# cvxopt/smcp

Measured on AMD Instinct MI355X. Metric: Newton KKT solves/sec, higher is better.
Workload: dtype f64; 1 GPU; synth50k nested block-arrow SDP n=50000, 8073 cliques, m=100; kktsolver=chol, n=50000, cliques=8073, m=100, blkval_doubles=2493568, update_doubles=10689536, parallelism=single

## Files before the change

### smcp_amd/build.py

```python
import os
import shutil
import subprocess
import sys

HERE = os.path.dirname(os.path.abspath(__file__))
CSRC = os.path.join(HERE, "csrc")
LIB = os.path.join(HERE, "libsmcp_amd.so")
SOURCES = ["capi.hip", "symbolic.cpp"]
DEPS = ["front_large.hip", "front_mfma.hip", "capi.hip", "kkt.hip", "kkt_qr.hip", "front_generic.hip", "front_mrc.hip", "front_edm.hip", "wgblas.hpp", "context.hpp", "symbolic.cpp",
        "symbolic.hpp", "../../include/smcp_amd.h"]


def _stale():
    if not os.path.exists(LIB):
        return True
    t = os.path.getmtime(LIB)
    for d in os.listdir(CSRC):
        if os.path.getmtime(os.path.join(CSRC, d)) > t:
            return True
    return os.path.getmtime(os.path.join(HERE, "..", "include", "smcp_amd.h")) > t


def build(force=False, verbose=True):
    if not force and not _stale():
        return LIB
    hipcc = shutil.which("hipcc") or "/opt/rocm/bin/hipcc"
    cmd = [hipcc, "--offload-arch=gfx950", "-O3", "-std=c++17", "-fPIC", "-shared",
           "-Wno-unused-result", "-Wno-unused-value", "-pthread", "-o", LIB] + [os.path.join(CSRC, s) for s in SOURCES]
    if os.environ.get("SMCP_STAMPS") == "1":
        cmd.insert(1, "-DSMCP_STAMPS")
    for flag in os.environ.get("SMCP_CXXFLAGS", "").split():
        cmd.insert(1, flag)
    if verbose:
        print(" ".join(cmd), file=sys.stderr)
    subprocess.check_call(cmd)
    return LIB


if __name__ == "__main__":
    build(force="--force" in sys.argv)
```

### smcp_amd/csrc/capi.hip

```cpp
#include <hip/hip_runtime.h>
#include <memory>
#include <unordered_map>

#include <algorithm>
#include <chrono>
#include <cstdio>
#include <cstring>
#include <map>
#include <new>
#include <atomic>
#include <thread>
#include <type_traits>
#include <vector>

#include "../../include/smcp_amd.h"
#include "context.hpp"
#include "switches.hpp"
#include "front_generic.hip"
#include "front_mfma.hip"
#include "front_large.hip"
#include "front_inv.hip"
#include "front_n16.hip"
#include "front_downfam.hip"
#include "front_fam.hip"
#include "front_fam2.hip"
#include "front_lfsp.hip"
#include "front_leafgram.hip"
#include "front_famt.hip"
#include "front_flow.hip"
#include "front_mrc.hip"
#include "front_edm.hip"

using namespace smcp;

#define HIPCHK(x)                                                                        \
  do {                                                                                   \
    hipError_t e_ = (x);                                                                 \
    if (e_ != hipSuccess) {                                                              \
      fprintf(stderr, "smcp_amd: HIP error %s at %s:%d\n", hipGetErrorString(e_), __FILE__, __LINE__); \
      return SMCP_EHIP;                                                                  \
    }                                                                                    \
  } while (0)

namespace {

enum {
  KID_chol_level = 0, KID_llt_level, KID_pinv_level, KID_gather_level, KID_completion_all,
  KID_hess_up_level, KID_hess_down_level, KID_hess_down_inv_all, KID_hess_up_inv_level, KID_scale_an,
  KID_factor_yaa, KID_trsm_fwd_level, KID_trsm_bwd_level, KID_amap, KID_aadj, KID_scatter_constraints,
  KID_dense_potrf, KID_dense_potrs, KID_vec_axpby, KID_axpby, KID_reduce_cliques, KID_reduce_final,
  KID_hess_up_mfma, KID_hess_down_mfma, KID_chol_mfma, KID_pinv_mfma, KID_prep_lk,
  KID_hess_up_mfma_hbm, KID_hess_down_mfma_hbm, KID_chol_mfma_hbm, KID_pinv_mfma_hbm,
  KID_gram_partial, KID_gram_reduce, KID_hess_up_pad,
  KID_lf_assemble, KID_lf_clear_upd, KID_lf_up1, KID_lf_up2, KID_lf_up3, KID_lf_down1, KID_lf_down2, KID_lf_down3,
  KID_lf_pinv1, KID_lf_pinv2, KID_lf_diag, KID_lf_chol_panel, KID_lf_chol_trail, KID_lf_pack_upd,
  KID_lf_prep_s, KID_lf_prep_row, KID_lf_prep_k, KID_factor_yaa_lds,
  KID_factor_inverse, KID_hess_down_inv_mfma, KID_hess_down_inv_mfma_hbm, KID_hess_up_inv_mfma, KID_hess_up_inv_mfma_hbm,
  KID_completion_mfma, KID_completion_mfma_hbm, KID_lf_copy_an, KID_lf_ri_an, KID_lf_dinv1, KID_lf_dinv2,
  KID_lf_uinv1, KID_lf_uinv2, KID_lf_completion, KID_hess_up_n16, KID_llt_mfma, KID_llt_mfma_hbm, KID_lf_llt,
  KID_hess_up_fam, KID_qr_rmul, KID_qr_dots, KID_qr_comb, KID_qr_small, KID_fam2_prep, KID_mid_chol, KID_lf_diag_inv, KID_lfsp_up, KID_lfsp_prep, KID_leaf_gram, KID_leaf_tables, KID_fam_sparse, KID_gram_diag128, KID_lf_assemble_lds, KID_fam_terms, KID_famt_prep, KID_lf_assemble_lds_dyn, KID_lf_zsp, KID_fam_terms_grp, KID_lf_assemble_fz, KID_factor_inverse_lds, KID_chol_flow,
  KID_mrc_diag, KID_mrc_rank, KID_mrc_reduce, KID_mrc_factor, KID_cut_signs, KID_cut_weights,
  KID_edm_rank, KID_edm_reduce, KID_edm_factor, KID_edm_dense, KID_hess_down_fam,
  KID_COUNT
};
const char* const KID_NAMES[KID_COUNT] = {
  "k_chol_level", "k_llt_level", "k_pinv_level", "k_gather_level", "k_completion_all",
  "k_hess_up_level", "k_hess_down_level", "k_hess_down_inv_all", "k_hess_up_inv_level", "k_scale_an",
  "k_factor_yaa", "k_trsm_fwd_level", "k_trsm_bwd_level", "k_amap", "k_aadj", "k_scatter_constraints",
  "k_dense_potrf", "k_dense_potrs", "k_vec_axpby", "k_axpby", "k_reduce_cliques", "k_reduce_final",
  "k_hess_up_mfma<true>", "k_hess_down_mfma<true>", "k_chol_mfma<true>", "k_pinv_mfma<true>", "k_prep_lk",
  "k_hess_up_mfma<false>", "k_hess_down_mfma<false>", "k_chol_mfma<false>", "k_pinv_mfma<false>",
  "k_gram_partial", "k_gram_reduce", "k_hess_up_pad",
  "k_lf_assemble", "k_lf_clear_upd", "k_lf_up1", "k_lf_up2", "k_lf_up3", "k_lf_down1", "k_lf_down2", "k_lf_down3",
  "k_lf_pinv1", "k_lf_pinv2", "k_lf_diag", "k_lf_chol_panel", "k_lf_chol_trail", "k_lf_pack_upd",
  "k_lf_prep_s", "k_lf_prep_row", "k_lf_prep_k", "k_factor_yaa_lds",
  "k_factor_inverse", "k_hess_down_inv_mfma<true>", "k_hess_down_inv_mfma<false>", "k_hess_up_inv_mfma<true>",
  "k_hess_up_inv_mfma<false>", "k_completion_mfma<true>", "k_completion_mfma<false>", "k_lf_copy_an", "k_lf_ri_an",
  "k_lf_dinv1", "k_lf_dinv2", "k_lf_uinv1", "k_lf_uinv2", "k_lf_completion", "k_hess_up_n16",
  "k_llt_mfma<true>", "k_llt_mfma<false>", "k_lf_llt", "k_hess_up_fam",
  "k_stack_trsm", "k_stack_dots", "k_stack_comb", "k_qr_small", "k_fam2_prep", "k_mid_chol", "k_lf_diag_inv", "k_lfsp_up", "k_lfsp_prep", "k_leaf_pairs", "k_leaf_tables", "k_fam_sparse", "k_gram_diag128", "k_lf_assemble_lds", "k_fam_terms", "k_famt_prep", "k_lf_assemble_lds_dyn", "k_lf_zsp", "k_fam_terms_grp", "k_lf_assemble_fz", "k_factor_inverse_lds", "k_chol_flow",
  "k_mrc_diag", "k_mrc_rank", "k_mrc_reduce", "k_mrc_factor", "k_cut_signs", "k_cut_weights",
  "k_edm_rank", "k_edm_reduce", "k_edm_factor", "k_edm_dense", "k_hess_down_fam"};

inline void note_launch(csp_ctx* c, int kid) {
  const hipError_t e = hipGetLastError();
  if (e != hipSuccess && !c->launch_err) {
    c->launch_err = (int)e;
    fprintf(stderr, "smcp_amd: launch of %s failed: %s\n", (kid >= 0 && kid < KID_COUNT) ? KID_NAMES[kid] : "?", hipGetErrorString(e));
  }
}
inline hipError_t end_call(csp_ctx* c) {
  hipError_t e = hipGetLastError();
  if (e == hipSuccess && c->launch_err) e = c->launch_err > 0 ? (hipError_t)c->launch_err : hipErrorLaunchFailure;
  c->launch_err = 0;
  return e;
}

__global__ void k_race_spin(long long ticks) {
  const long long t0 = wall_clock64();
  for (int it = 0; it < (1 << 22) && wall_clock64() - t0 < ticks; ++it) __builtin_amdgcn_s_sleep(8);
}
struct RaceInject {
  std::atomic<uint64_t> state{0};
  std::atomic<int64_t> injected{0};
  std::atomic<int> max_us{200};
  std::atomic<int> drop_joins{0};
  bool on() const { return state.load(std::memory_order_relaxed) != 0; }
  void seed(uint64_t s) { state.store(s ? (s * 0x9E3779B97F4A7C15ull) | 1ull : 0ull); }
  uint64_t next() {
    uint64_t x = state.load(std::memory_order_relaxed);
    x ^= x << 13; x ^= x >> 7; x ^= x << 17;
    state.store(x | 1ull, std::memory_order_relaxed);
    return x;
  }
};
inline RaceInject& race_inject() {
  static RaceInject r;
  static const bool init = [] { const char* e = sw_str("SMCP_RACE"); if (e && atoll(e) > 0) r.seed((uint64_t)atoll(e)); return true; }();
  (void)init;
  return r;
}
inline void race_delay(hipStream_t s, bool always = true) {
  RaceInject& r = race_inject();
  if (!r.on()) return;
  const uint64_t x = r.next();
  if (!always && (x >> 40) % 4 != 0) return;
  const long long us = 5 + (long long)((x >> 16) % (uint64_t)std::max(1, r.max_us.load(std::memory_order_relaxed) - 4));
  hipLaunchKernelGGL(k_race_spin, dim3(1), dim3(64), 0, s, us * 100);
  r.injected.fetch_add(1, std::memory_order_relaxed);
}

inline unsigned sync_event_flags() {
  static int sys = -1;
  if (sys < 0) { const char* e = sw_str("SMCP_EVENT_SYSFENCE"); sys = (e && e[0] == '1') ? 1 : 0; }
  return sys ? hipEventDisableTiming : (hipEventDisableTiming | hipEventReleaseToDevice);
// ... 1061 lines not shown
  if (!D.sp_rt) {
    if (dev_alloc(&D.sp_rt, std::max<int64_t>(c->S.updlen(), 1), D.bytes)) return false;
    if (dev_alloc(&D.sp_mk, std::max<int64_t>(c->S.blklen(), 1), D.bytes)) return false;
  }
  MfmaArgs b = a;
  b.sp_rt = D.sp_rt; b.sp_mk = D.sp_mk;
  if (D.sp_fac_gen != D.fac_gen || D.sp_lk_gen != D.lk_gen) {
    MfmaArgs p = b;
    p.t.lev = D.lfsp_list;
    launch(c, KID_lfsp_prep, k_lfsp_prep, dim3((unsigned)D.lfsp_cnt), dim3(256), st, p, a.ysc, D.sp_rt, D.sp_mk);
    D.sp_fac_gen = D.fac_gen; D.sp_lk_gen = D.lk_gen;
  }
  static int gdiv = -1;
  if (gdiv < 0) { const char* e = sw_str("SMCP_LFSP_G"); gdiv = e ? std::max(1, atoi(e)) : 1; }
  const int g = std::max(1, (nrhs + gdiv - 1) / gdiv);
  const dim3 grid(g, cnt), blk(256);
  const bool grouped = grp && grp->ngroups > 0;
  MfmaArgs bg = b;
  if (grouped) { bg.grp_ptr = grp->ptr; bg.grp_list = grp->list; }
  const dim3 ggrid(g, grouped ? grp->ngroups : cnt);
  static const int gocc = sw_int("SMCP_LFSP_OCC", 2);
  if (grouped && gocc == 1) {
    if (exact) {
      launch(c, KID_lfsp_up, k_lfsp_up<8, 4, 1, 3, 1, false, true>, grid, blk, st, b, U, ldu);
      launch(c, KID_lfsp_up, k_lfsp_up<8, 4, 2, 1, 1, false, true, true>, ggrid, blk, st, bg, U, ldu);
      launch(c, KID_lfsp_up, k_lfsp_up<8, 4, 4, 4, 1, false, true>, grid, blk, st, b, U, ldu);
    } else {
      launch(c, KID_lfsp_up, k_lfsp_up<8, 4, 1, 3, 1, false, false>, grid, blk, st, b, U, ldu);
      launch(c, KID_lfsp_up, k_lfsp_up<8, 4, 2, 1, 1, false, false, true>, ggrid, blk, st, bg, U, ldu);
      launch(c, KID_lfsp_up, k_lfsp_up<8, 4, 4, 4, 1, false, false>, grid, blk, st, b, U, ldu);
    }
    return true;
  }
  if (exact) {
    launch(c, KID_lfsp_up, k_lfsp_up<8, 4, 1, 3, 1, false, true>, grid, blk, st, b, U, ldu);
    if (grouped) launch(c, KID_lfsp_up, k_lfsp_up<8, 4, 2, 2, 1, false, true, true>, ggrid, blk, st, bg, U, ldu);
    else launch(c, KID_lfsp_up, k_lfsp_up<8, 4, 2, 2, 1, false, true>, grid, blk, st, b, U, ldu);
    launch(c, KID_lfsp_up, k_lfsp_up<8, 4, 4, 4, 1, false, true>, grid, blk, st, b, U, ldu);
  } else {
    launch(c, KID_lfsp_up, k_lfsp_up<8, 4, 1, 3, 1, false, false>, grid, blk, st, b, U, ldu);
    if (grouped) launch(c, KID_lfsp_up, k_lfsp_up<8, 4, 2, 2, 1, false, false, true>, ggrid, blk, st, bg, U, ldu);
    else launch(c, KID_lfsp_up, k_lfsp_up<8, 4, 2, 2, 1, false, false>, grid, blk, st, b, U, ldu);
    launch(c, KID_lfsp_up, k_lfsp_up<8, 4, 4, 4, 1, false, false>, grid, blk, st, b, U, ldu);
  }
  return true;
}
bool lfsp_dynamic_ok(csp_ctx* c, const MfmaArgs& a) {
  static int on = -1;
  if (on < 0) { const char* e = sw_str("SMCP_LFSP"); on = (e && e[0] == '0') ? 0 : 1; }
  const DeviceCtx& D = c->D;
  return on && a.kc_ptr && a.ymode == 2 && a.ysc && D.kc_maxlist_large > 0 && D.kc_maxlist_large <= LFSP_ECAP && D.lfsp_cnt;
}

void hess_up_fast(csp_ctx* c, double* U, int nrhs, int64_t ldu, const double* ysc, int ymode, hipStream_t st, int set = 0,
                  int64_t sparse_j0 = -1, const int32_t* ids = nullptr, int64_t lev_lo = 0, int64_t lev_hi = -1,
                  const double* yroot = nullptr) {
  MfmaArgs a0 = mfma_args(c, ysc, ymode, nrhs);
  const bool sparse = sparse_j0 >= 0 && c->D.kc_ptr;
  if (sparse) {
    a0.kc_ptr = c->D.kc_ptr; a0.kc_off = c->D.kc_off; a0.kc_val = c->D.kc_val; a0.kc_ids = ids;
    a0.kc_stride = (int)(c->D.m + 1); a0.kc_j0 = (int)sparse_j0;
  }
  const bool groups_on = sparse && set == 0 && c->lfsp_any_groups && c->D.lfsp_skip && lfsp_dynamic_ok(c, a0);
  const bool fgroups_on = sparse && set == 0 && c->famt_any_groups && c->D.famt_skip && !famt_disabled() && !fam2_disabled() && c->D.lg_request &&
                          c->D.kc_ij && a0.ymode == 2 && a0.ysc && c->D.fam_maxterms <= FAMT_TCAP / 2 &&
                          c->D.cnnz <= (int64_t)4 * c->S.nsn * std::max<int64_t>(1, c->D.m);
  if (groups_on || fgroups_on) a0.chskip = groups_on && fgroups_on ? c->D.both_skip : (groups_on ? c->D.lfsp_skip : c->D.famt_skip);
  c->fz_live = false;
  {
    static int fzenv = -1;
    if (fzenv < 0) { const char* e = sw_str("SMCP_FZ"); fzenv = (e && e[0] == '0') ? 0 : 1; }
    bool want = fzenv && sparse && (set == 0 || (set == 1 && c->fz_set1_ok)) && lev_lo == 0 && lev_hi < 0 && !fgroups_on && c->D.fz_ok && !famt_disabled() && !fam2_disabled() &&
                c->D.lg_request && c->D.kc_ij && a0.ymode == 2 && a0.ysc && famt_terms_ok(c->D) &&
                c->D.cnnz <= (int64_t)4 * c->S.nsn * std::max<int64_t>(1, c->D.m) && !use_generic(c) && use_large() && c->D.gp_tptr;
    int famlevels = 0, nofill = 0;
    if (want) {
      for (int64_t l = 0; l < c->S.nlev; ++l)
        for_level_classes(c, l, a0, [&](bool lds, MfmaArgs a, int cnt, size_t, int) {
          if (lds && a.nS > 0 && a.level > 0) ++famlevels;
          if (!lds && (size_t)a.level < c->fz_levels.size() && c->fz_levels[(size_t)a.level] && !(a.nchmax > 0 && lf_assemble_fills(c, a, cnt, nrhs, true))) { want = false; ++nofill; }
        }, set);
      if (famlevels != 1) want = false;
    }
    if (want) { a0.fz_on = 1; a0.fz_no = c->D.fz_no; }
    static int occ = -1;
    if (occ < 0) occ = sw_on("SMCP_OCC", 0);
    if (occ && sparse)
      fprintf(stderr, "fz: want %d famlevels %d nofill %d nlev %d (env %d set %d lev %d..%d fgroups %d fz_ok %d famt_off %d fam2_off %d lg_request %d kc_ij %d ymode %d ysc %d maxterms %d cnnz %lld nsn %lld m %lld generic %d nrhs %d)\n",
              (int)want, famlevels, nofill, (int)c->S.nlev, fzenv, set, (int)lev_lo, (int)lev_hi, (int)fgroups_on, (int)c->D.fz_ok, (int)famt_disabled(), (int)fam2_disabled(), (int)c->D.lg_request,
              c->D.kc_ij != nullptr, a0.ymode, a0.ysc != nullptr, (int)c->D.fam_maxterms, (long long)c->D.cnnz, (long long)c->S.nsn, (long long)c->D.m, (int)use_generic(c), nrhs);
  }
  auto dense_input_on = [&](MfmaArgs& a, int cnt, double* Ub, int nr, hipStream_t s) {
    if (!sparse) return;
    for (int r0 = 0; r0 < nr; r0 += 65535) {
      MfmaArgs af = a;
      af.kc_j0 = a.kc_j0 + r0;
      const int64_t pan = (int64_t)(a.nnmax + a.namax) * a.nnmax;
      const int nz = (int)std::max<int64_t>(1, std::min<int64_t>(std::min<int64_t>(a.nnmax, 64), pan / 16384));
      launch(c, KID_scatter_constraints, k_panel_fill, dim3(cnt, std::min(65535, nr - r0), nz), dim3(256), s, af, Ub + (int64_t)r0 * ldu, ldu);
    }
    a.kc_ptr = nullptr;
  };
  auto dense_input = [&](MfmaArgs& a, int cnt) { dense_input_on(a, cnt, U, nrhs, st); };
  for (int64_t l = lev_lo; l < (lev_hi < 0 ? c->S.nlev : lev_hi); ++l) {
    for_level_classes(c, l, a0, [&](bool lds, MfmaArgs a, int cnt, size_t bytes, int thr) {
      static int fam_minrhs = -1;
      if (fam_minrhs < 0) { const char* e = sw_str("SMCP_FAM_MINRHS"); fam_minrhs = e ? atoi(e) : 1; }
      if (lds && a.nS > 0 && (sparse || nrhs >= fam_minrhs)) {
        const int nS = a.nS;
        a.nS = 0;
        if (a.level > 0) {
          MfmaArgs af = a;
          af.t.lev = a.t.lev + (cnt - nS);
          if (fgroups_on && (size_t)l < c->famt_grp.size() && c->famt_grp[(size_t)l].ngroups > 0) {
            af.grp_ptr = c->famt_grp[(size_t)l].ptr; af.grp_list = c->famt_grp[(size_t)l].list; af.famt_ngrp = c->famt_grp[(size_t)l].ngroups;
          }
          if (!try_fam(c, af, nS, nrhs, U, ldu, st)) {
            fprintf(stderr, "smcp_amd: family kernel not launchable (LDS budget or attribute)\n");
            if (!c->launch_err) c->launch_err = -1;
          }
        }
        cnt -= nS;
        if (cnt == 0) return;
      }
      int g = rhs_groups(cnt, nrhs, lds ? 2048 : 1024);
      if (lds) {
        hipStream_t ls = st;
        static int oldk = -1;
        if (oldk < 0) { const char* e = sw_str("SMCP_OLDLDS"); oldk = (e && e[0] == '1') ? 1 : 0; }
        size_t pbytes = (size_t)pad_layout(a.nnmax, a.namax, a.nchmax, a.panmax, a.pkmax, a.plansum).total * sizeof(double);
        if (!oldk && try_n16(c, a, cnt, nrhs, U, ldu, ls)) {
        } else if (!oldk && pbytes <= LDS_LIMIT) {
          dense_input_on(a, cnt, U, nrhs, ls);
          launch_lds(c, KID_hess_up_pad, k_hess_up_pad, dim3(cnt, g), dim3(pbytes > 48 * 1024 ? 512 : 256), pbytes, ls, a, U, ldu);
        } else {
          dense_input_on(a, cnt, U, nrhs, ls);
          launch_lds(c, KID_hess_up_mfma, k_hess_up_mfma<true>, dim3(cnt, g), dim3(thr), bytes, ls, a, U, ldu);
        }
      } else if (use_large() && c->D.gp_tptr) {
        {
          const csp_ctx::LfspGroups* grp = groups_on && (size_t)l < c->lfsp_grp.size() && c->lfsp_grp[(size_t)l].ngroups > 0 ? &c->lfsp_grp[(size_t)l] : nullptr;
          if (sparse && try_lfsp(c, a, cnt, nrhs, U, ldu, st, grp)) return;
          if (grp) {
            fprintf(stderr, "smcp_amd: sparse-input sweep of a grouped level not launchable\n");
            if (!c->launch_err) c->launch_err = -1;
          }
        }
        static int split_min = -1;
        if (split_min < 0) { const char* e = sw_str("SMCP_RHS_SPLIT"); split_min = e ? atoi(e) : 16; }
        static int parts = -1;
        if (parts < 0) { const char* e = sw_str("SMCP_RHS_PARTS"); parts = (e && e[0] == '3') ? 3 : 2; }
        const int ncu_split = c->D.ncu;
        static int dynsplit = -1;
        if (dynsplit < 0) { const char* e = sw_str("SMCP_ALDS_DYN"); const char* f = sw_str("SMCP_RHS_SPLIT_DYN"); dynsplit = ((e && e[0] == '0') || (f && f[0] == '1')) ? 1 : 0; }
        if (dynsplit && split_min > 0 && a.nchmax > 0 && nrhs >= split_min && (int64_t)cnt * nrhs > ncu_split && Fork::enabled()) {
          auto part = [&](int r0, int nr, hipStream_t s) {
            MfmaArgs ap = a;
            ap.nrhs = nr;
            ap.t.upd += (int64_t)r0 * a.t.updlen;
            ap.t.updp += (int64_t)r0 * a.t.updplen;
            ap.t.tmp += (int64_t)r0 * a.t.tmplen;
            ap.kc_j0 = a.kc_j0 + r0;
            dense_input_on(ap, cnt, U + (int64_t)r0 * ldu, nr, s);
            lf_up(c, ap, cnt, nr, U + (int64_t)r0 * ldu, ldu, s);
          };
          if (parts == 3 && nrhs >= 3) {
            const int h1 = nrhs / 3, h2 = (2 * nrhs) / 3;
            Fork f0(c, st, 0);
            part(h2, nrhs - h2, f0.s);
            Fork f1(c, st, 1);
            part(h1, h2 - h1, f1.s);
            part(0, h1, st);
            return;
          }
          const int h = nrhs / 2;
          Fork f(c, st, 0);
          part(h, nrhs - h, f.s);
          part(0, h, st);
          return;
        }
        static int zsp = -1;
        if (zsp < 0) { const char* e = sw_str("SMCP_ZSP"); zsp = (e && e[0] == '0') ? 0 : 1; }
        if (zsp && sparse && c->D.kc_sorted && a.nchmax == 0 && a.namax == 0 && lf_sym_split(a.nnmin) && a.nnmax <= LF_ZSP_MAXNN) {
          const int ntN = tiles64(a.nnmax);
          launch_lds(c, KID_lf_zsp, k_lf_zsp, dim3(a.nnmax, cnt, nrhs), dim3(256), (size_t)a.nnmax * sizeof(double), st, a, U, ldu);
          LAUNCH_PD(c, KID_lf_up2, k_lf_up2, dim3(umax1(ntN * (ntN + 1) / 2), cnt, nrhs), dim3(256), st, a, U, ldu);
          return;
        }
        const bool fzlev = c->fz_live && (size_t)a.level < c->fz_levels.size() && c->fz_levels[(size_t)a.level];
        if (sparse && a.nchmax > 0 && lf_assemble_fills(c, a, cnt, nrhs, fzlev)) {
          lf_up(c, a, cnt, nrhs, U, ldu, st, true);
          return;
        }
        dense_input(a, cnt);
        if (yroot && a.namax == 0 && a.nnmax <= ROOT_FUSED_MAXNN && root_fused()) {
          if (a.nchmax > 0) lf_assemble(c, a, cnt, nrhs, U, ldu, 0, st, true);
          const int ntN = tiles64(a.nnmax);
          LAUNCH_PD(c, KID_lf_up1, k_lf_root1, dim3(umax1(ntN * ntN), cnt, nrhs), dim3(256), st, a, U, ldu, yroot);
          return;
        }
        lf_up(c, a, cnt, nrhs, U, ldu, st);
      }
      else { dense_input(a, cnt); launch_lds(c, KID_hess_up_mfma_hbm, k_hess_up_mfma<false>, dim3(cnt, nrhs), dim3(thr), 0, st, a, U, ldu); }
    }, set);
  }
}
void gather_set(csp_ctx* c, int set, const double* x, int64_t ldx, int nrhs, double* updbase, hipStream_t st) {
  TreeArgs a = tree_args(c);
  const LevelSet& LS = c->sets[set];
  for (int64_t l = c->S.nlev - 1; l >= 0; --l) {
    const LevelClass& L = LS.lvl[l];
    const int cnt = (int)(L.nI + L.nII);
    if (!cnt) continue;
    a.lev = LS.lev2 + LS.off[l];
    launch(c, KID_gather_level, k_gather_level, dim3(cnt, nrhs, gather_parts(std::max(L.namaxI, L.namaxII), (int64_t)cnt * nrhs, c->D.ncu)), dim3(NT), st, a, x, ldx, updbase);
  }
}
int down_fam_maxrhs() {
  static int v = -1;
  if (v < 0) v = std::min(65535, std::max(0, sw_int("SMCP_DOWN_FAM", 1)));
  return v;
}
void launch_down_fam(csp_ctx* c, const MfmaArgs& a, int cnt, int nrhs, double* U, int64_t ldu, hipStream_t st,
                     const int32_t* lone = nullptr, int nlone = 0, int lnn = 0, int lna = 0) {
  const int nfmax = std::max(a.famnn + a.famna, lnn + lna), cpan = (a.famcnn + a.famcna) * a.famcnn;
  const size_t bytes = down_fam_lds_bytes(nfmax, cpan);
  const int pnat = (std::max(std::max(a.famna, lna), 1) + 15) / 16, cnat = (std::max(a.famcna, 1) + 15) / 16;
  const dim3 grid(cnt + nlone, nrhs), blk(256);
  switch (2 * pnat + cnat) {
    case 3: launch_lds(c, KID_hess_down_fam, k_hess_down_fam<1, 1>, grid, blk, bytes, st, a, U, ldu, nfmax, cpan, cnt, lone); break;
    case 4: launch_lds(c, KID_hess_down_fam, k_hess_down_fam<1, 2>, grid, blk, bytes, st, a, U, ldu, nfmax, cpan, cnt, lone); break;
    case 5: launch_lds(c, KID_hess_down_fam, k_hess_down_fam<2, 1>, grid, blk, bytes, st, a, U, ldu, nfmax, cpan, cnt, lone); break;
    case 6: launch_lds(c, KID_hess_down_fam, k_hess_down_fam<2, 2>, grid, blk, bytes, st, a, U, ldu, nfmax, cpan, cnt, lone); break;
    case 7: launch_lds(c, KID_hess_down_fam, k_hess_down_fam<3, 1>, grid, blk, bytes, st, a, U, ldu, nfmax, cpan, cnt, lone); break;
    case 8: launch_lds(c, KID_hess_down_fam, k_hess_down_fam<3, 2>, grid, blk, bytes, st, a, U, ldu, nfmax, cpan, cnt, lone); break;
    case 9: launch_lds(c, KID_hess_down_fam, k_hess_down_fam<4, 1>, grid, blk, bytes, st, a, U, ldu, nfmax, cpan, cnt, lone); break;
    default: launch_lds(c, KID_hess_down_fam, k_hess_down_fam<4, 2>, grid, blk, bytes, st, a, U, ldu, nfmax, cpan, cnt, lone); break;
  }
}
void hess_down_fast(csp_ctx* c, double* U, int nrhs, int64_t ldu, const double* ysc, int ymode, hipStream_t st, int set = 0,
                    const double* yroot = nullptr) {
  MfmaArgs a0 = mfma_args(c, ysc, ymode, nrhs);
  MfmaArgs fam1 = a0;
  int nfam1 = 0;
  for (int64_t l = c->S.nlev - 1; l >= 0; --l)
    for_level_classes(c, l, a0, [&](bool lds, MfmaArgs a, int cnt, size_t bytes, int thr) {
      if (lds && a.nS > 0 && ymode == 0 && nrhs <= down_fam_maxrhs()) {
        const int nS = a.nS;
        a.nS = 0;
        MfmaArgs af = a;
        af.t.lev = a.t.lev + (cnt - nS);
        cnt -= nS;
        if (a.level > 1) launch_down_fam(c, af, nS, nrhs, U, ldu, st);
        else if (a.level == 1) { fam1 = af; nfam1 = nS; }
        else if (nfam1 > 0) {
          const bool fits = cnt > 0 && a.nnmax <= 16 && a.namax <= 64;
          launch_down_fam(c, fam1, nfam1, nrhs, U, ldu, st, fits ? a.t.lev : nullptr, fits ? cnt : 0, fits ? a.nnmax : 0, fits ? a.namax : 0);
// ... 1823 lines not shown
```

### smcp_amd/csrc/switches.hpp

```cpp
#pragma once
#include <cstdio>
#include <cstdlib>
#include <cstring>
#include <string>

extern char** environ;

namespace smcp {

struct Switch { const char* name; const char* dflt; const char* doc; };

static const Switch SWITCHES[] = {
  {"SMCP_GENERIC", "0", "1: any-size fixed-order kernels of front_generic.hip for every tree operation (as CSP_TUNE_DETERMINISTIC)"},
  {"SMCP_LARGE", "1", "0: no tiled large-front kernels (fronts beyond LDS take the one-workgroup HBM kernels)"},
  {"SMCP_NOCACHE", "0", "1: nothing derived from (L, Y) is reused between calls"},
  {"SMCP_FORK", "1", "0: no side streams, everything on the caller's stream"},
  {"SMCP_AUX_PRIO", "1", "0: side stream 0 (few-workgroup chains) at default instead of highest priority"},
  {"SMCP_AUX_PRIO1", "1", "0: side stream 1 (filler work) at default instead of lowest priority"},
  {"SMCP_EVENT_SYSFENCE", "0", "1: internal events with the default system-scope release (12 us per hand-over instead of 7)"},
  {"SMCP_SCALING_OVERLAP", "1", "0: csp_cholesky_projected_inverse as its three steps one after the other"},
  {"SMCP_CHOL_PREP", "1", "0: k_prep_lk in a launch of its own instead of inside k_chol_mfma (narrow supernodes)"},
  {"SMCP_FAC_PARTIAL", "1", "0: chol(Y_AA) of the family children always formed by the fused scaling point"},
  {"SMCP_MID", "1", "0: per-step kernels instead of k_mid_chol / k_lf_diag_inv for fronts of at most 272 rows"},
  {"SMCP_TRTRI", "1", "0: block-row triangular inversion of large fronts instead of recursive doubling"},
  {"SMCP_N16", "1", "0: no shape-specialised k_hess_up_n16"},
  {"SMCP_OLDLDS", "0", "1: k_hess_up_mfma<true> instead of the padded / n16 kernels"},
  {"SMCP_DOWN_W", "1", "0: k_hess_down_mfma instead of the one-wave k_hess_down_w"},
  {"SMCP_DOWN_FAM", "1", "most right-hand sides of a root -> leaves sweep that take the one-launch family kernel k_hess_down_fam (0: never; the per-level k_hess_down_w launches)"},
  {"SMCP_FAM", "1", "0: no family kernels (per-level sweeps with the update exchange through HBM)"},
  {"SMCP_FAM2", "1", "0: no sparse-input family kernels (k_fam_sparse, k_fam_terms): k_hess_up_fam"},
  {"SMCP_FAMT", "1", "0: no entry-driven family sweep k_fam_terms (k_fam_sparse instead)"},
  {"SMCP_FZ", "1", "0: the family parents' packed updates go through HBM (k_fam_terms writes, the extend-add reads) instead of being formed by k_lf_assemble_fz"},
  {"SMCP_FAMT_GROUP", "1", "0: no sibling groups of family parents (k_fam_terms_grp)"},
  {"SMCP_LFSP", "1", "0: dense phases instead of the sparse-input sweep k_lfsp_up of childless large fronts"},
  {"SMCP_LFSP_GROUP", "1", "0: no sibling groups in k_lfsp_up"},
  {"SMCP_ZSP", "1", "0: dense first phase of wide childless fronts instead of k_lf_zsp"},
  {"SMCP_LEAFGRAM", "1", "0: never the closed-form Gram blocks of the family children (k_leaf_tables / k_leaf_pairs)"},
  {"SMCP_LG_SIDE", "1", "0: leaf Gram blocks after the sweep on the caller's stream instead of beside the top phases"},
  {"SMCP_GRAM_EARLY", "0", "1: the Gram chunks of the levels 0 / 1 rows on the side branch beside the top fronts' phase kernels (measured slower: 3.37 against 3.22 ms per step)"},
  {"SMCP_LG_EARLY", "1", "0: leaf Gram blocks beside the phase kernels of the top fronts instead of from the start of the sweep"},
  {"SMCP_FACI_LDS", "1", "0: inverse Y_AA factors of the small fronts by block rows against HBM (k_factor_inverse) instead of in LDS"},
  {"SMCP_FZ_TAIL", "1", "0: every (front, right-hand side) pair of the fused extend-add is one workgroup's task, also in a thin last round"},
  {"SMCP_GRAM", "1", "0: reference (two-sweep) formulation of the Schur complement instead of the Gram formulation"},
  {"SMCP_SCM", "1", "0: column-sparse constraints swept like the others (no SCMcolumn2 route)"},
  {"SMCP_TRSM_MM", "1", "0: csp_trsm through the generic level kernels instead of tile products"},
  {"SMCP_ALDS", "1", "0: extend-add of large fronts by gather plan only (no LDS streaming kernel)"},
  {"SMCP_ALDS_DYN", "1", "0: one workgroup per (front, right-hand side) instead of the task-drawing grid"},
  {"SMCP_ALDS_FILL", "1", "0: k_panel_fill builds the input panels instead of the extend-add (sgn 3)"},
  {"SMCP_ASM", "plan", "t: tiled extend-add kernel instead of the gather plan"},
  {"SMCP_ROOT_FUSED", "0", "1: fused two-product sweep of fronts without separator (Y_NN explicit: condition squared; studies only)"},
  {"SMCP_PD", "0", "1: four-wave tile products everywhere (no sixteen-wave shape for small launches)"},
  {"SMCP_POTRF_OLD", "0", "1: generic one-workgroup dense Cholesky"},
  {"SMCP_FLOW", "1", "0: no one-launch blocked Cholesky with in-launch tile dataflow (front_flow.hip): per-step kernels for dense matrices / single fronts beyond 272 rows"},
  {"SMCP_FLOW_WG", "112", "workgroups of that launch (at most 112: four launches fit the chip side by side)"},
  {"SMCP_POTRS_OLD", "0", "1: generic one-workgroup dense solve"},
  {"SMCP_POTRS_STEPS", "0", "1: per-block launches of the dense solve instead of k_dense_potrs_one"},
  {"SMCP_POTRF_DEFER", "1", "0: kkt_schur_factor factors H at once even under deferred status"},
  {"SMCP_QR_TRSM", "mfma", "f: vector-FMA substitution kernel of kkt_qr instead of the MFMA one"},
  {"SMCP_FTHR_CHOL", "128", "threads of k_chol_mfma on the leaf class"},
  {"SMCP_FTHR_PINV", "256", "threads of k_pinv_mfma on the leaf class"},
  {"SMCP_FTHR_YAA", "64", "threads of k_factor_yaa_lds on the leaf class"},
  {"SMCP_FTHR_YAA_MID", "256", "threads of k_factor_yaa_lds on separator blocks of 33 .. 64 rows"},
  {"SMCP_N16_THR_LEAF", "128", "threads of k_hess_up_n16 for one or two right-hand sides on childless fronts"},
  {"SMCP_DIAG_THREADS", "512", "threads of k_lf_diag"},
  {"SMCP_POTRF_THREADS", "1024", "threads of k_dense_potrf_small"},
  {"SMCP_FZ_THREADS", "1024", "threads of k_lf_assemble_fz (512: eight waves, no register spills, slower)"},
  {"SMCP_PD_WGS", "1", "largest launch, in workgroups per CU, that takes the sixteen-wave tile shape"},
  {"SMCP_ALDS_Z", "0", "workgroups per (front, right-hand side) of the LDS extend-add (0: automatic)"},
  {"SMCP_RHS_SPLIT", "16", "fewest right-hand sides for the two-stream split of a large-front sweep (plain extend-add launch only)"},
  {"SMCP_RHS_PARTS", "2", "parts of that split (2 or 3)"},
  {"SMCP_RHS_SPLIT_DYN", "0", "1: the split also with the task-drawing extend-add"},
  {"SMCP_FAM_MINRHS", "1", "fewest dense right-hand sides for the family kernel"},
  {"SMCP_FAMT_G", "0", "right-hand-side slices per family of k_fam_terms (0: cost model)"},
  {"SMCP_FAM2_STAG", "0", "stagger of k_fam_sparse's groups (studies)"},
  {"SMCP_FAMT_MEAN", "36", "entry-driven family sweeps (k_fam_terms, fused extend-add) up to this many entries per (family, constraint) list ON AVERAGE (lists up to 384 entries, in chunks); beyond: the dense family sweep"},
  {"SMCP_LFSP_OCC", "2", "waves per SIMD the grouped update phase of k_lfsp_up is compiled for (1: 512 registers, no spills; 2: 256, ~100 spilled)"},
  {"SMCP_LFSP_G", "1", "right-hand sides per workgroup of k_lfsp_up"},
  {"SMCP_GRAM_NW", "16", "waves per workgroup of k_gram_diag128 (4, 8 or 16)"},
  {"SMCP_GRAM_MINCHUNK", "512", "fewest stack rows per workgroup of the Gram accumulation"},
  {"SMCP_UPDP_PAD", "0", "doubles of padding between the packed exchange buffers of consecutive right-hand sides"},
  {"SMCP_QR_PASSES", "0", "Cholesky-QR passes of kkt_qr (0: decided by the deviation test)"},
// ... 43 lines not shown
```

Before: 324.6 KKT solves/s.

## Add resident one-launch family kernel for single-RHS dense up-sweep with level-0 ride-along

Adds k_hess_up_fam1, which handles a family parent and its up to eight children in one workgroup. Each wave processes children in registers with MFMA and accumulates their updates into the parent's packed front in LDS through LDS atomics, prefetching the next child's data while the current one computes. For dense sweeps with at most SMCP_UP_FAM right-hand sides (default 1), the leftover level-0 cliques that sit outside any family are deferred and issued as extra blocks of the same launch. This is meant to remove a separate level-0 launch and the HBM round trip of child updates. The cost is a narrower shape envelope and more complex dispatch, with a fallback path when the kernel cannot be used.

```diff
diff --git a/smcp_amd/build.py b/smcp_amd/build.py
--- a/smcp_amd/build.py
+++ b/smcp_amd/build.py
@@ -7,7 +7,7 @@
 CSRC = os.path.join(HERE, "csrc")
 LIB = os.path.join(HERE, "libsmcp_amd.so")
 SOURCES = ["capi.hip", "symbolic.cpp"]
-DEPS = ["front_large.hip", "front_mfma.hip", "capi.hip", "kkt.hip", "kkt_qr.hip", "front_generic.hip", "front_mrc.hip", "front_edm.hip", "wgblas.hpp", "context.hpp", "symbolic.cpp",
+DEPS = ["front_large.hip", "front_mfma.hip", "capi.hip", "kkt.hip", "kkt_qr.hip", "front_generic.hip", "front_mrc.hip", "front_edm.hip", "front_downfam.hip", "front_upfam.hip", "wgblas.hpp", "context.hpp", "symbolic.cpp",
         "symbolic.hpp", "../../include/smcp_amd.h"]
 
 
diff --git a/smcp_amd/csrc/capi.hip b/smcp_amd/csrc/capi.hip
--- a/smcp_amd/csrc/capi.hip
+++ b/smcp_amd/csrc/capi.hip
@@ -23,6 +23,7 @@
 #include "front_n16.hip"
 #include "front_downfam.hip"
 #include "front_fam.hip"
+#include "front_upfam.hip"
 #include "front_fam2.hip"
 #include "front_lfsp.hip"
 #include "front_leafgram.hip"
@@ -60,7 +61,7 @@
   KID_lf_uinv1, KID_lf_uinv2, KID_lf_completion, KID_hess_up_n16, KID_llt_mfma, KID_llt_mfma_hbm, KID_lf_llt,
   KID_hess_up_fam, KID_qr_rmul, KID_qr_dots, KID_qr_comb, KID_qr_small, KID_fam2_prep, KID_mid_chol, KID_lf_diag_inv, KID_lfsp_up, KID_lfsp_prep, KID_leaf_gram, KID_leaf_tables, KID_fam_sparse, KID_gram_diag128, KID_lf_assemble_lds, KID_fam_terms, KID_famt_prep, KID_lf_assemble_lds_dyn, KID_lf_zsp, KID_fam_terms_grp, KID_lf_assemble_fz, KID_factor_inverse_lds, KID_chol_flow,
   KID_mrc_diag, KID_mrc_rank, KID_mrc_reduce, KID_mrc_factor, KID_cut_signs, KID_cut_weights,
-  KID_edm_rank, KID_edm_reduce, KID_edm_factor, KID_edm_dense, KID_hess_down_fam,
+  KID_edm_rank, KID_edm_reduce, KID_edm_factor, KID_edm_dense, KID_hess_down_fam, KID_hess_up_fam1,
   KID_COUNT
 };
 const char* const KID_NAMES[KID_COUNT] = {
@@ -80,7 +81,7 @@
   "k_llt_mfma<true>", "k_llt_mfma<false>", "k_lf_llt", "k_hess_up_fam",
   "k_stack_trsm", "k_stack_dots", "k_stack_comb", "k_qr_small", "k_fam2_prep", "k_mid_chol", "k_lf_diag_inv", "k_lfsp_up", "k_lfsp_prep", "k_leaf_pairs", "k_leaf_tables", "k_fam_sparse", "k_gram_diag128", "k_lf_assemble_lds", "k_fam_terms", "k_famt_prep", "k_lf_assemble_lds_dyn", "k_lf_zsp", "k_fam_terms_grp", "k_lf_assemble_fz", "k_factor_inverse_lds", "k_chol_flow",
   "k_mrc_diag", "k_mrc_rank", "k_mrc_reduce", "k_mrc_factor", "k_cut_signs", "k_cut_weights",
-  "k_edm_rank", "k_edm_reduce", "k_edm_factor", "k_edm_dense", "k_hess_down_fam"};
+  "k_edm_rank", "k_edm_reduce", "k_edm_factor", "k_edm_dense", "k_hess_down_fam", "k_hess_up_fam1"};
 
 inline void note_launch(csp_ctx* c, int kid) {
   const hipError_t e = hipGetLastError();
@@ -1248,6 +1249,43 @@
   return on && a.kc_ptr && a.ymode == 2 && a.ysc && D.kc_maxlist_large > 0 && D.kc_maxlist_large <= LFSP_ECAP && D.lfsp_cnt;
 }
 
+int up_fam_maxrhs() {
+  static int v = -1;
+  if (v < 0) v = std::min(65535, std::max(0, sw_int("SMCP_UP_FAM", 1)));
+  return v;
+}
+template <int PNAT, int CNAT>
+bool launch_up_fam1_t(csp_ctx* c, const MfmaArgs& a, dim3 grid, size_t bytes, double* U, int64_t ldu, hipStream_t st, int nfmax, int cpan, int cnt, const int32_t* lone) {
+  static bool attr = false;
+  if (bytes > 64 * 1024 && !attr) {
+    if (hipFuncSetAttribute((const void*)k_hess_up_fam1<PNAT, CNAT>, hipFuncAttributeMaxDynamicSharedMemorySize, 160 * 1024 - 1024) != hipSuccess) return false;
+    attr = true;
+  }
+  if (a.ysc == c->D.fac) complete_fac(c, st);
+  launch_lds(c, KID_hess_up_fam1, k_hess_up_fam1<PNAT, CNAT>, grid, dim3(256), bytes, st, a, U, ldu, nfmax, cpan, cnt, lone);
+  return true;
+}
+bool launch_up_fam1(csp_ctx* c, const MfmaArgs& a, int cnt, int nrhs, double* U, int64_t ldu, hipStream_t st,
+                    const int32_t* lone = nullptr, int nlone = 0, int lnn = 0, int lna = 0) {
+  if (a.famnn > 16 || a.famna > 64 || a.famcnn > 16 || a.famcna > 32 || lnn > 16 || lna > 64 || nrhs > 65535) return false;
+  const int nfmax = std::max(a.famnn + a.famna, lnn + lna), cpan = (a.famcnn + a.famcna) * a.famcnn;
+  const size_t bytes = down_fam_lds_bytes(nfmax, cpan);
+  if (bytes > LDS_LIMIT) return false;
+  const int pnat = (std::max(std::max(a.famna, lna), 1) + 15) / 16, cnat = (std::max(a.famcna, 1) + 15) / 16;
+  const dim3 grid(cnt + nlone, nrhs);
+  switch (2 * pnat + cnat) {
+    case 3: return launch_up_fam1_t<1, 1>(c, a, grid, bytes, U, ldu, st, nfmax, cpan, cnt, lone);
+    case 4: return launch_up_fam1_t<1, 2>(c, a, grid, bytes, U, ldu, st, nfmax, cpan, cnt, lone);
+    case 5: return launch_up_fam1_t<2, 1>(c, a, grid, bytes, U, ldu, st, nfmax, cpan, cnt, lone);
+    case 6: return launch_up_fam1_t<2, 2>(c, a, grid, bytes, U, ldu, st, nfmax, cpan, cnt, lone);
+    case 7: return launch_up_fam1_t<3, 1>(c, a, grid, bytes, U, ldu, st, nfmax, cpan, cnt, lone);
+    case 8: return launch_up_fam1_t<3, 2>(c, a, grid, bytes, U, ldu, st, nfmax, cpan, cnt, lone);
+    case 9: return launch_up_fam1_t<4, 1>(c, a, grid, bytes, U, ldu, st, nfmax, cpan, cnt, lone);
+    case 10: return launch_up_fam1_t<4, 2>(c, a, grid, bytes, U, ldu, st, nfmax, cpan, cnt, lone);
+  }
+  return false;
+}
+
 void hess_up_fast(csp_ctx* c, double* U, int nrhs, int64_t ldu, const double* ysc, int ymode, hipStream_t st, int set = 0,
                   int64_t sparse_j0 = -1, const int32_t* ids = nullptr, int64_t lev_lo = 0, int64_t lev_hi = -1,
                   const double* yroot = nullptr) {
@@ -1298,7 +1336,25 @@
     a.kc_ptr = nullptr;
   };
   auto dense_input = [&](MfmaArgs& a, int cnt) { dense_input_on(a, cnt, U, nrhs, st); };
-  for (int64_t l = lev_lo; l < (lev_hi < 0 ? c->S.nlev : lev_hi); ++l) {
+  const int64_t lev_end = lev_hi < 0 ? c->S.nlev : lev_hi;
+  const bool up1 = !sparse && nrhs <= up_fam_maxrhs();
+  struct { MfmaArgs a; int cnt = 0; size_t bytes = 0; int thr = 0; } out0;
+  auto small_level = [&](MfmaArgs& a, int cnt, size_t bytes, int thr) {
+    const int g = rhs_groups(cnt, nrhs, 2048);
+    hipStream_t ls = st;
+    static int oldk = -1;
+    if (oldk < 0) { const char* e = sw_str("SMCP_OLDLDS"); oldk = (e && e[0] == '1') ? 1 : 0; }
+    size_t pbytes = (size_t)pad_layout(a.nnmax, a.namax, a.nchmax, a.panmax, a.pkmax, a.plansum).total * sizeof(double);
+    if (!oldk && try_n16(c, a, cnt, nrhs, U, ldu, ls)) {
+    } else if (!oldk && pbytes <= LDS_LIMIT) {
+      dense_input_on(a, cnt, U, nrhs, ls);
+      launch_lds(c, KID_hess_up_pad, k_hess_up_pad, dim3(cnt, g), dim3(pbytes > 48 * 1024 ? 512 : 256), pbytes, ls, a, U, ldu);
+    } else {
+      dense_input_on(a, cnt, U, nrhs, ls);
+      launch_lds(c, KID_hess_up_mfma, k_hess_up_mfma<true>, dim3(cnt, g), dim3(thr), bytes, ls, a, U, ldu);
+    }
+  };
+  for (int64_t l = lev_lo; l < lev_end; ++l) {
     for_level_classes(c, l, a0, [&](bool lds, MfmaArgs a, int cnt, size_t bytes, int thr) {
       static int fam_minrhs = -1;
       if (fam_minrhs < 0) { const char* e = sw_str("SMCP_FAM_MINRHS"); fam_minrhs = e ? atoi(e) : 1; }
@@ -1311,6 +1367,12 @@
           if (fgroups_on && (size_t)l < c->famt_grp.size() && c->famt_grp[(size_t)l].ngroups > 0) {
             af.grp_ptr = c->famt_grp[(size_t)l].ptr; af.grp_list = c->famt_grp[(size_t)l].list; af.famt_ngrp = c->famt_grp[(size_t)l].ngroups;
           }
+          const bool took1 = up1 && !af.famt_ngrp &&
+                             launch_up_fam1(c, af, nS, nrhs, U, ldu, st, out0.cnt ? out0.a.t.lev : nullptr, out0.cnt, out0.cnt ? out0.a.nnmax : 0, out0.cnt ? out0.a.namax : 0);
+          if (!took1 && out0.cnt) small_level(out0.a, out0.cnt, out0.bytes, out0.thr);
+          out0.cnt = 0;
+          if (took1) {
+          } else
           if (!try_fam(c, af, nS, nrhs, U, ldu, st)) {
             fprintf(stderr, "smcp_amd: family kernel not launchable (LDS budget or attribute)\n");
             if (!c->launch_err) c->launch_err = -1;
@@ -1318,22 +1380,13 @@
         }
         cnt -= nS;
         if (cnt == 0) return;
+        if (up1 && a.level == 0 && l + 1 < lev_end && a.nnmax <= 16 && a.namax <= 64) {
+          const LevelClass& L1 = set ? c->sets[set].lvl[l + 1] : c->lvl[l + 1];
+          if (L1.nI > 0 && L1.nS > 0) { out0.a = a; out0.cnt = cnt; out0.bytes = bytes; out0.thr = thr; return; }
+        }
       }
-      int g = rhs_groups(cnt, nrhs, lds ? 2048 : 1024);
-      if (lds) {
-        hipStream_t ls = st;
-        static int oldk = -1;
-        if (oldk < 0) { const char* e = sw_str("SMCP_OLDLDS"); oldk = (e && e[0] == '1') ? 1 : 0; }
-        size_t pbytes = (size_t)pad_layout(a.nnmax, a.namax, a.nchmax, a.panmax, a.pkmax, a.plansum).total * sizeof(double);
-        if (!oldk && try_n16(c, a, cnt, nrhs, U, ldu, ls)) {
-        } else if (!oldk && pbytes <= LDS_LIMIT) {
-          dense_input_on(a, cnt, U, nrhs, ls);
-          launch_lds(c, KID_hess_up_pad, k_hess_up_pad, dim3(cnt, g), dim3(pbytes > 48 * 1024 ? 512 : 256), pbytes, ls, a, U, ldu);
-        } else {
-          dense_input_on(a, cnt, U, nrhs, ls);
-          launch_lds(c, KID_hess_up_mfma, k_hess_up_mfma<true>, dim3(cnt, g), dim3(thr), bytes, ls, a, U, ldu);
-        }
-      } else if (use_large() && c->D.gp_tptr) {
+      if (lds) small_level(a, cnt, bytes, thr);
+      else if (use_large() && c->D.gp_tptr) {
         {
           const csp_ctx::LfspGroups* grp = groups_on && (size_t)l < c->lfsp_grp.size() && c->lfsp_grp[(size_t)l].ngroups > 0 ? &c->lfsp_grp[(size_t)l] : nullptr;
           if (sparse && try_lfsp(c, a, cnt, nrhs, U, ldu, st, grp)) return;
@@ -1399,6 +1452,10 @@
       }
       else { dense_input(a, cnt); launch_lds(c, KID_hess_up_mfma_hbm, k_hess_up_mfma<false>, dim3(cnt, nrhs), dim3(thr), 0, st, a, U, ldu); }
     }, set);
+  }
+  if (out0.cnt) {
+    fprintf(stderr, "smcp_amd: level-0 cliques handed to a family launch that was never issued\n");
+    if (!c->launch_err) c->launch_err = -1;
   }
 }
 void gather_set(csp_ctx* c, int set, const double* x, int64_t ldx, int nrhs, double* updbase, hipStream_t st) {
diff --git a/smcp_amd/csrc/front_upfam.hip b/smcp_amd/csrc/front_upfam.hip
--- /dev/null
+++ b/smcp_amd/csrc/front_upfam.hip
@@ -0,0 +1,345 @@
+#include <hip/hip_runtime.h>
+
+namespace smcp {
+
+__device__ inline double up_fam_ysc(const double* ys, int ymode, int m, int kk, int na) {
+  if (m >= na || kk >= na) return 0.0;
+  if (ymode == 1) return m >= kk ? ys[m + kk * na] : ys[kk + m * na];
+  if (ymode == 2) return kk >= m ? ys[kk + m * na] : 0.0;
+  return m >= kk ? ys[m + kk * na] : 0.0;
+}
+
+struct UpPre { double vp[4], vl[4]; int rel; };
+__device__ inline void up_fam_fetch(UpPre& p, const MfmaArgs& a, const CliqueDesc& d, const double* U, int lane) {
+  const int pan = (d.nn + d.na) * d.nn;
+  const double* P = U + d.blk;
+  const double* LK = a.LK + d.blk;
+#pragma unroll
+  for (int h = 0; h < 4; ++h) {
+    const int e = 64 * h + lane;
+    p.vp[h] = e < pan ? P[(unsigned)e] : 0.0;
+    p.vl[h] = e < pan ? LK[(unsigned)e] : 0.0;
+  }
+  p.rel = lane < d.na ? a.t.relidx[d.rel + lane] : 0;
+}
+__device__ inline void up_fam_commit(const DownStage& st, const UpPre& p, const CliqueDesc& d, int lane) {
+  const int pan = (d.nn + d.na) * d.nn;
+#pragma unroll
+  for (int h = 0; h < 4; ++h) {
+    const int e = 64 * h + lane;
+    if (e < pan) { st.P[e] = p.vp[h]; st.LK[e] = p.vl[h]; }
+  }
+  if (lane < d.na) st.rel[lane] = p.rel;
+}
+
+template <int NATC, class F>
+__device__ inline void up_fam_child(const MfmaArgs& a, const DownStage& st, const CliqueDesc& cd, double* Pc, double* zs, int nfz, int lane, F loaded) {
+  const int l15 = lane & 15, kq = lane >> 4;
+  const int nnc = cd.nn, nac = cd.na, nfc = nnc + nac;
+  const int ksnc = (nnc + 3) >> 2, ksac = (nac + 3) >> 2;
+  const int ymode = a.ymode;
+  const d4 zero4 = {0.0, 0.0, 0.0, 0.0};
+  double kreg[NATC][4], bdreg[4], fnn[4], fan[NATC][4];
+  int rm[NATC];
+  wave_sync();
+#pragma unroll
+  for (int s = 0; s < 4; ++s) {
+    const int kk = kq + 4 * s;
+    bdreg[s] = (l15 < nnc && kk <= l15) ? st.LK[l15 + kk * nfc] : 0.0;
+    fnn[s] = (l15 < nnc && kk < nnc) ? st.P[max(l15, kk) + min(l15, kk) * nfc] : 0.0;
+#pragma unroll
+    for (int t = 0; t < NATC; ++t) {
+      const int m = 16 * t + l15;
+      const bool in = m < nac && kk < nnc;
+      kreg[t][s] = in ? st.LK[nnc + m + kk * nfc] : 0.0;
+      fan[t][s] = in ? st.P[nnc + m + kk * nfc] : 0.0;
+    }
+  }
+#pragma unroll
+  for (int t = 0; t < NATC; ++t) {
+    const int m = 16 * t + l15;
+    rm[t] = m < nac ? st.rel[m] : -1;
+  }
+  wave_sync();
+  loaded();
+  d4 accE[NATC], accT = zero4;
+#pragma unroll
+  for (int t = 0; t < NATC; ++t) {
+    accE[t] = zero4;
+#pragma unroll
+    for (int s = 0; s < 4; ++s)
+      if (s < ksnc) fmma(accE[t], kreg[t][s], fnn[s]);
+  }
+#pragma unroll
+  for (int s = 0; s < 4; ++s)
+    if (s < ksnc) fmma(accT, bdreg[s], fnn[s]);
+  double ev[NATC][4], xv[NATC][4];
+#pragma unroll
+  for (int t = 0; t < NATC; ++t)
+#pragma unroll
+    for (int rr = 0; rr < 4; ++rr) {
+      ev[t][rr] = fan[t][rr] - 0.5 * accE[t][rr];
+      xv[t][rr] = fan[t][rr] - accE[t][rr];
+    }
+#pragma unroll
+  for (int tm = 0; tm < NATC; ++tm)
+#pragma unroll
+    for (int tn = 0; tn <= tm; ++tn) {
+      if (16 * tm >= nac) continue;
+      d4 acc = zero4;
+#pragma unroll
+      for (int s = 0; s < 4; ++s)
+        if (s < ksnc) {
+          fmma(acc, kreg[tm][s], ev[tn][s]);
+          fmma(acc, ev[tm][s], kreg[tn][s]);
+        }
+      const int ri = rm[tm];
+#pragma unroll
+      for (int rr = 0; rr < 4; ++rr) {
+        const int n = 16 * tn + kq + 4 * rr;
+        if (ri >= 0 && n < nac && 16 * tm + l15 >= n) unsafeAtomicAdd(&zs[pk_low(ri, st.rel[n], nfz)], -acc[rr]);
+      }
+    }
+  d4 accG[NATC], accN = zero4;
+#pragma unroll
+  for (int t = 0; t < NATC; ++t) {
+    accG[t] = zero4;
+#pragma unroll
+    for (int s = 0; s < 4; ++s)
+      if (s < ksnc) fmma(accG[t], xv[t][s], bdreg[s]);
+  }
+#pragma unroll
+  for (int s = 0; s < 4; ++s)
+    if (s < ksnc) fmma(accN, accT[s], bdreg[s]);
+#pragma unroll
+  for (int rr = 0; rr < 4; ++rr) {
+    const int jn = kq + 4 * rr;
+    if (l15 < nnc && jn <= l15) Pc[l15 + jn * nfc] = accN[rr];
+  }
+  if (!ymode) {
+#pragma unroll
+    for (int t = 0; t < NATC; ++t)
+#pragma unroll
+      for (int rr = 0; rr < 4; ++rr) {
+        const int m = 16 * t + l15, n = kq + 4 * rr;
+        if (m < nac && n < nnc) Pc[(nnc + m) + n * nfc] = accG[t][rr];
+      }
+    return;
+  }
+#pragma unroll
+  for (int t = 0; t < NATC; ++t)
+#pragma unroll
+    for (int rr = 0; rr < 4; ++rr) {
+      const int m = 16 * t + l15, n = kq + 4 * rr;
+      if (m < nac && n < nnc) st.P[m + n * nac] = accG[t][rr];
+    }
+  wave_sync();
+  double gv[4 * NATC];
+#pragma unroll
+  for (int s2 = 0; s2 < 4 * NATC; ++s2) {
+    const int kk = kq + 4 * s2;
+    gv[s2] = (kk < nac && l15 < nnc) ? st.P[kk + l15 * nac] : 0.0;
+  }
+  const double* ys = a.ysc + cd.upd;
+#pragma unroll
+  for (int t = 0; t < NATC; ++t) {
+    if (16 * t >= nac) continue;
+    double yc[4 * NATC];
+#pragma unroll
+    for (int s2 = 0; s2 < 4 * NATC; ++s2) yc[s2] = up_fam_ysc(ys, ymode, 16 * t + l15, kq + 4 * s2, nac);
+    d4 acc = zero4;
+#pragma unroll
+    for (int s2 = 0; s2 < 4 * NATC; ++s2)
+      if (s2 < ksac && !(ymode == 2 && s2 < 4 * t) && !(ymode == 3 && s2 >= 4 * (t + 1)))
+        fmma(acc, yc[s2], gv[s2]);
+#pragma unroll
+    for (int rr = 0; rr < 4; ++rr) {
+      const int m = 16 * t + l15, n = kq + 4 * rr;
+      if (m < nac && n < nnc) Pc[(nnc + m) + n * nfc] = acc[rr];
+    }
+  }
+  wave_sync();
+}
+
+template <int PNAT, int CNAT>
+__global__ void __launch_bounds__(256, 4) k_hess_up_fam1(MfmaArgs a, double* u, int64_t ldu, int nfmax, int cpan, int nfam, const int32_t* lone) {
+  extern __shared__ double zs[];
+  const int tid = threadIdx.x;
+  const int lane = tid & 63, l15 = lane & 15, kq = lane >> 4;
+  const int wave = __builtin_amdgcn_readfirstlane((int)(threadIdx.x >> 6));
+  const int k = (int)blockIdx.x < nfam ? a.t.lev[blockIdx.x] : lone[(int)blockIdx.x - nfam];
+  const CliqueDesc d = a.t.cl[k];
+  const int nn = d.nn, na = d.na, nf = nn + na;
+  const int nch = (int)blockIdx.x < nfam ? d.chend - d.chbeg : 0;
+  if (nch > 8 && tid == 0) atomicCAS(a.t.info, 0, -7);
+  double* const U = u + (int64_t)blockIdx.y * ldu;
+  double* const P = U + d.blk;
+  double* const UkP = a.t.updp + (int64_t)blockIdx.y * a.t.updplen + d.updp;
+  const int ymode = a.ymode;
+  const int ksn = (nn + 3) >> 2, ksa = (na + 3) >> 2;
+  const d4 zero4 = {0.0, 0.0, 0.0, 0.0};
+  const bool has0 = wave < nch, has1 = wave + 4 < nch;
+  const CliqueDesc dc0 = a.t.cl[has0 ? a.t.chidx[d.chbeg + wave] : k];
+  const CliqueDesc dc1 = a.t.cl[has1 ? a.t.chidx[d.chbeg + wave + 4] : k];
+  const DownStage st = down_fam_stage_of(zs + nfmax * (nfmax + 1) / 2, wave, cpan);
+  if (has0) down_fam_stage(st, a, dc0, U, lane);
+  {
+    double v[8];
+#pragma unroll
+    for (int c = 0; c < 4; ++c) {
+      const int j = wave + 4 * c;
+#pragma unroll
+      for (int h = 0; h < 2; ++h) {
+        const int i = j + lane + 64 * h;
+        v[2 * c + h] = (j < nn && i < nf) ? P[i + j * nf] : 0.0;
+      }
+    }
+#pragma unroll
+    for (int c = 0; c < 4; ++c) {
+      const int j = wave + 4 * c;
+#pragma unroll
+      for (int h = 0; h < 2; ++h) {
+        const int i = j + lane + 64 * h;
+        if (j < nn && i < nf) zs[pk_low(i, j, nf)] = v[2 * c + h];
+      }
+    }
+    for (int e = pk_low(nn, nn, nf) + tid; e < nf * (nf + 1) / 2; e += 256) zs[e] = 0.0;
+  }
+  __syncthreads();
+  const bool pre1 = has1 && (dc1.nn + dc1.na) * dc1.nn <= 256;
+  UpPre pre;
+  if (has0) up_fam_child<CNAT>(a, st, dc0, U + dc0.blk, zs, nf, lane, [&]() { if (pre1) up_fam_fetch(pre, a, dc1, U, lane); });
+  if (has1) {
+    if (pre1) up_fam_commit(st, pre, dc1, lane);
+    else down_fam_stage(st, a, dc1, U, lane);
+    up_fam_child<CNAT>(a, st, dc1, U + dc1.blk, zs, nf, lane, []() {});
+  }
+  __syncthreads();
+  const int gw = wave;
+  const double* const lk = a.LK + d.blk;
+  double bdP[4], kt[PNAT][4], kPm[4] = {0.0, 0.0, 0.0, 0.0};
+#pragma unroll
+  for (int s = 0; s < 4; ++s) {
+    const int kk = kq + 4 * s;
+    bdP[s] = (l15 < nn && kk <= l15) ? lk[l15 + kk * nf] : 0.0;
+#pragma unroll
+    for (int t = 0; t < PNAT; ++t) {
+      const int m = 16 * t + l15;
+      kt[t][s] = (t <= gw && m < na && kk < nn) ? lk[(nn + m) + kk * nf] : 0.0;
+      if (t == gw) kPm[s] = kt[t][s];
+    }
+  }
+  double ev[PNAT][4], evm[4] = {0.0, 0.0, 0.0, 0.0}, xvm[4] = {0.0, 0.0, 0.0, 0.0};
+  d4 accT = zero4;
+  {
+    double fnn[4];
+#pragma unroll
+    for (int s = 0; s < 4; ++s) {
+      const int kr = kq + 4 * s;
+      fnn[s] = (kr < nn && l15 < nn) ? zs[pk_low(max(kr, l15), min(kr, l15), nf)] : 0.0;
+    }
+#pragma unroll
+    for (int t = 0; t < PNAT; ++t) {
+#pragma unroll
+      for (int rr = 0; rr < 4; ++rr) ev[t][rr] = 0.0;
+      if (t <= gw && 16 * t < na) {
+        double fan[4];
+        const int m = 16 * t + l15;
+#pragma unroll
+        for (int s = 0; s < 4; ++s) fan[s] = (m < na && kq + 4 * s < nn) ? zs[pk_low(nn + m, kq + 4 * s, nf)] : 0.0;
+        d4 acc = zero4;
+#pragma unroll
+        for (int s = 0; s < 4; ++s)
+          if (s < ksn) fmma(acc, kt[t][s], fnn[s]);
+#pragma unroll
+        for (int rr = 0; rr < 4; ++rr) ev[t][rr] = fan[rr] - 0.5 * acc[rr];
+        if (t == gw) {
+#pragma unroll
+          for (int rr = 0; rr < 4; ++rr) { evm[rr] = ev[t][rr]; xvm[rr] = fan[rr] - acc[rr]; }
+        }
+      }
+    }
+    if (gw == 0) {
+#pragma unroll
+      for (int s = 0; s < 4; ++s)
+        if (s < ksn) fmma(accT, bdP[s], fnn[s]);
+    }
+  }
+  __syncthreads();
+  if (gw < PNAT && 16 * gw < na) {
+    const int m = 16 * gw + l15;
+#pragma unroll
+    for (int tn = 0; tn < PNAT; ++tn) {
+      if (tn > gw) continue;
+      d4 acc = zero4;
+#pragma unroll
+      for (int s = 0; s < 4; ++s)
+        if (s < ksn) {
+          fmma(acc, kPm[s], ev[tn][s]);
+          fmma(acc, evm[s], kt[tn][s]);
+        }
+      double uv[4];
+#pragma unroll
+      for (int rr = 0; rr < 4; ++rr) {
+        const int n = 16 * tn + kq + 4 * rr;
+        uv[rr] = (m >= n && m < na) ? zs[pk_low(nn + m, nn + n, nf)] : 0.0;
+      }
+#pragma unroll
+      for (int rr = 0; rr < 4; ++rr) {
+        const int n = 16 * tn + kq + 4 * rr;
+        if (m >= n && m < na) UkP[n * na - ((n * (n - 1)) >> 1) + (m - n)] = uv[rr] - acc[rr];
+      }
+    }
+    d4 acc = zero4;
+#pragma unroll
+    for (int s = 0; s < 4; ++s)
+      if (s < ksn) fmma(acc, xvm[s], bdP[s]);
+#pragma unroll
+    for (int rr = 0; rr < 4; ++rr) {
+      const int n = kq + 4 * rr;
+      if (m < na && n < nn) {
+        if (ymode) zs[pk_low(nn + m, n, nf)] = acc[rr];
+        else P[(nn + m) + n * nf] = acc[rr];
+      }
+    }
+  }
+  if (gw == 0) {
+    d4 acc = zero4;
+#pragma unroll
+    for (int s = 0; s < 4; ++s)
+      if (s < ksn) fmma(acc, accT[s], bdP[s]);
+#pragma unroll
+    for (int rr = 0; rr < 4; ++rr) {
+      const int jn = kq + 4 * rr;
+      if (l15 < nn && jn <= l15) P[l15 + jn * nf] = acc[rr];
+    }
+  }
+  if (!ymode) return;
+  __syncthreads();
+  if (gw < PNAT && 16 * gw < na) {
+    const double* ys = a.ysc + d.upd;
+    const int m = 16 * gw + l15;
+    d4 acc = zero4;
+#pragma unroll
+    for (int s0 = 0; s0 < 4 * PNAT; s0 += 8) {
+      double yv[8], gv[8];
+#pragma unroll
+      for (int s2 = s0; s2 < s0 + 8 && s2 < 4 * PNAT; ++s2) {
+        const int kk = kq + 4 * s2;
+        yv[s2 - s0] = up_fam_ysc(ys, ymode, m, kk, na);
+        gv[s2 - s0] = (kk < na && l15 < nn) ? zs[pk_low(nn + kk, l15, nf)] : 0.0;
+      }
+#pragma unroll
+      for (int s2 = s0; s2 < s0 + 8 && s2 < 4 * PNAT; ++s2)
+        if (s2 < ksa && !(ymode == 2 && s2 < 4 * gw) && !(ymode == 3 && s2 >= 4 * (gw + 1)))
+          fmma(acc, yv[s2 - s0], gv[s2 - s0]);
+    }
+#pragma unroll
+    for (int rr = 0; rr < 4; ++rr) {
+      const int n = kq + 4 * rr;
+      if (m < na && n < nn) P[(nn + m) + n * nf] = acc[rr];
+    }
+  }
+}
+
+}
diff --git a/smcp_amd/csrc/switches.hpp b/smcp_amd/csrc/switches.hpp
--- a/smcp_amd/csrc/switches.hpp
+++ b/smcp_amd/csrc/switches.hpp
@@ -27,6 +27,7 @@
   {"SMCP_OLDLDS", "0", "1: k_hess_up_mfma<true> instead of the padded / n16 kernels"},
   {"SMCP_DOWN_W", "1", "0: k_hess_down_mfma instead of the one-wave k_hess_down_w"},
   {"SMCP_DOWN_FAM", "1", "most right-hand sides of a root -> leaves sweep that take the one-launch family kernel k_hess_down_fam (0: never; the per-level k_hess_down_w launches)"},
+  {"SMCP_UP_FAM", "1", "most dense right-hand sides of a leaves -> root sweep that take the resident family kernel k_hess_up_fam1, the level-0 cliques outside the families riding along (0: never; k_hess_up_fam and a launch of their own for those cliques)"},
   {"SMCP_FAM", "1", "0: no family kernels (per-level sweeps with the update exchange through HBM)"},
   {"SMCP_FAM2", "1", "0: no sparse-input family kernels (k_fam_sparse, k_fam_terms): k_hess_up_fam"},
   {"SMCP_FAMT", "1", "0: no entry-driven family sweep k_fam_terms (k_fam_sparse instead)"},
```

New measurement: 336.3 KKT solves/s, median of 6. 1.04x the previous value.
